# Angtian/VoGE

Measured on AMD Instinct MI355X. Metric: forward+backward frames/sec at 512^2, 50k Gaussians; ray-trace HBM GB/s vs peak, higher is better.
Workload: dtype f32; 1 GPU; cfg3_50k_512: 50000 random Gaussians (scalar sigmas), 512x512, K=40, max_point_per_bin=-1, fwd+bwd (grads to verts, sigmas, colors); launch=hip graph replay, 4 consecutive steps per graph launch, parallelism=1 gpu

## Files before the change

voge_amd/csrc/fragment_bwd.hip:

```cpp
#include "composite_core.h"

namespace voge {

#ifndef VOGE_FB_NE
#define VOGE_FB_NE 128
#endif
constexpr int kFbNE = VOGE_FB_NE;
#ifndef VOGE_FB_GW
#define VOGE_FB_GW 4
#endif
#ifndef VOGE_FB_GH
#define VOGE_FB_GH 3
#endif
constexpr int kFbGW = VOGE_FB_GW, kFbGH = VOGE_FB_GH, kFbG = kFbGW * kFbGH;
static_assert(kFbG <= 64 && (kFbGW & (kFbGW - 1)) == 0, "a group's pixels are the lanes of one wave; GW a power of two");
#ifdef VOGE_FB_TIMES
constexpr int kFbTimesWaves = 1 << 16;
__device__ unsigned long long g_fb_times[kFbTimesWaves][8];
__device__ unsigned long long g_fb_tab[kFbTimesWaves][4];
__device__ unsigned long long g_fb_wall[kFbTimesWaves][2];
#define FB_T0() const unsigned long long fb_w0_ = __builtin_amdgcn_s_memrealtime(); unsigned long long fb_t_ = __builtin_readcyclecounter(), fb_acc_[6] = {0, 0, 0, 0, 0, 0}
#define FB_TICK(i) do { const unsigned long long n_ = __builtin_readcyclecounter(); fb_acc_[i] += n_ - fb_t_; fb_t_ = n_; } while (0)
#define FB_TOUT() do { if (threadIdx.x == 0 && blockIdx.x < kFbTimesWaves) { for (int i_ = 0; i_ < 6; ++i_) g_fb_times[blockIdx.x][i_] = fb_acc_[i_]; g_fb_times[blockIdx.x][6] = 1ull; g_fb_wall[blockIdx.x][0] = fb_w0_; g_fb_wall[blockIdx.x][1] = __builtin_amdgcn_s_memrealtime(); } } while (0)
#else
#define FB_T0() do {} while (0)
#define FB_TICK(i) do {} while (0)
#define FB_TOUT() do {} while (0)
#endif

template <int NV4, int NS>
struct FragBwdLds {
  static constexpr int kRows = NS * 64 + 4 * kFbG;
  WaveTable<kFbNE, NV4> tab;
  float len[kRows], sp[kRows], E[kRows], u[kRows];
  float r[kRows];
  unsigned spare[kFbG];
};

#ifndef VOGE_FB_ABL
#define VOGE_FB_ABL 0
#endif
#ifndef VOGE_FB_WPE
#define VOGE_FB_WPE 4
#endif
template <int SRC, int C, int NS, typename OffT, bool ISO, bool NOAD, bool DIAG = false>
__global__ void __launch_bounds__(64) __attribute__((amdgpu_waves_per_eu(NS == 4 ? 2 : (ISO ? VOGE_FB_WPE : 3))))
fragment_bwd_kernel(const float4 *__restrict__ rec, const float *__restrict__ rays,
                        const float *__restrict__ colors, const int32_t *__restrict__ idx, const int32_t *__restrict__ cnt,
                        const float *__restrict__ weight, const float *__restrict__ act, const float *__restrict__ len,
                        const float *__restrict__ dsd, const float *__restrict__ rgb, const float *__restrict__ wsum,
                        const float *__restrict__ bg, const float thr, const float *__restrict__ g_img, const long gs_pix,
                        const long gs_c, const float *__restrict__ g_hitlen, const float occ,
                        const int P, const long nrows, const int W, const int K, const long Nattr,
                        float *__restrict__ acc ) {
  static_assert(NS == 2 || NS == 4, "a lane owns one or two aligned pairs of slots");
  static_assert(!DIAG || (!ISO && NOAD && C <= 4), "the per-axis form keeps no act / dsd");
  constexpr int NV4 = SRC == 0 ? (ISO ? 2 : (DIAG ? 3 : 4)) : (ISO ? 1 : (DIAG ? 2 : 3)), NACC = 4 * NV4;
  constexpr int NRC = ISO ? 1 : (DIAG ? 2 : 3);
  auto sum_add = [&](const int key, const int c, const float v) { unsafeAtomicAdd(acc + NACC * (size_t)key + c, v); };
  __shared__ __attribute__((aligned(16))) FragBwdLds<NV4, NS> L;
  float *const Llen = L.len, *const Lsp = L.sp, *const LE = L.E, *const Lu = L.u, *const LR = L.r;
  const int lane = threadIdx.x;
  FB_T0();
  const int blocks_x = (W + kFbGW - 1) / kFbGW;
  const long blk = blockIdx.x;
  const int x0 = (int)(blk % blocks_x) * kFbGW;
  const long y0 = (blk / blocks_x) * kFbGH;
  const bool vec = (K % NS) == 0;
  const int gx = x0 + (lane & (kFbGW - 1));
  const long gy = y0 + lane / kFbGW;
  const bool pv = lane < kFbG && gx < W && gy < nrows;
  const int lead_g = pv ? min(K, max(0, cnt[gy * W + gx])) : 0;
  const int need = (lead_g + NS - 1) / NS;
  const int incl = wave_incl_scan(need, lane);
  if (__builtin_amdgcn_readlane(incl, 63) == 0) return;
  wt_clear(L.tab, lane);
  int pc = 0, off = 0;
  while (pc < kFbG) {
    PackLane pk;
    int npm;
    const int pe = pack_round(need, incl, kFbG, lane, pc, off, pk, npm);
    off = __builtin_amdgcn_readlane(incl, pe - 1);
    pc = pe;
    if (npm == 0) continue;
    FB_TICK(0);
    const bool on = pk.p >= 0;
    const int q = on ? lane - pk.s0 : 0, LP = on ? pk.np : 1;
    const int lead = __shfl(lead_g, on ? pk.p : 0, 64);
    const int k0 = NS * q;
    const OffT pix = on ? (OffT)((y0 + pk.p / kFbGW) * W + x0 + (pk.p & (kFbGW - 1))) : (OffT)0;
    const OffT fb = (pix * (OffT)K + (OffT)k0) * (OffT)4;
    const int r0 = NS * pk.s0 + 4 * pk.ord, RS = NS * LP + 4;
    const int d0 = on ? r0 + 2 + k0 : 2;
    int id[NS];
    float wv[NS], lm[NS], sm[NS], em[NS], gwv[NS];
    bool live[NS];
#pragma unroll
    for (int a = 0; a < NS; ++a) {
      id[a] = -1; wv[a] = 0.f; lm[a] = VOGE_SENT_LEN; sm[a] = 1e-5f; em[a] = 0.f; gwv[a] = 0.f;
      live[a] = on && (k0 + a < lead);
    }
    const float3 dv = at_bytes<float3>(rays, pix * (OffT)12);
    const float dx = on ? dv.x : 0.f, dy = on ? dv.y : 0.f, dz = on ? dv.z : 0.f;
    float4 rc[NS][NRC];
    float av[NS], dv2[NS];
#pragma unroll
    for (int a = 0; a < NS; ++a) { av[a] = 0.f; dv2[a] = 0.f; }
    {
      int idr[NS];
      float wr[NS], lr[NS], ar[NS], dr[NS], gr_[NS];
#pragma unroll
      for (int a = 0; a < NS; ++a) { idr[a] = -1; wr[a] = 0.f; lr[a] = VOGE_SENT_LEN; ar[a] = 0.f; dr[a] = 0.f; gr_[a] = 0.f; }
      const bool gw_wide = SRC == 1 && g_img != nullptr && vec && gs_c == 1 && gs_pix == (long)K;
      if (vec) {
#pragma unroll
        for (int h2 = 0; h2 < NS / 2; ++h2) {
          const OffT fo = fb + (OffT)(8 * h2);
          const int2 i2 = at_bytes<int2>(idx, fo);
          const v2f w2 = at_bytes<v2f>(weight, fo), l2 = at_bytes<v2f>(len, fo);
          idr[2 * h2] = i2.x; idr[2 * h2 + 1] = i2.y; wr[2 * h2] = w2.x; wr[2 * h2 + 1] = w2.y; lr[2 * h2] = l2.x; lr[2 * h2 + 1] = l2.y;
          if (!NOAD) {
            const v2f a2 = at_bytes<v2f>(act, fo), d2 = at_bytes<v2f>(dsd, fo);
            ar[2 * h2] = a2.x; ar[2 * h2 + 1] = a2.y; dr[2 * h2] = d2.x; dr[2 * h2 + 1] = d2.y;
          }
          if (gw_wide) {
            const v2f g2 = at_bytes<v2f>(g_img, fo);
            gr_[2 * h2] = g2.x; gr_[2 * h2 + 1] = g2.y;
          }
        }
      } else {
#pragma unroll
        for (int a = 0; a < NS; ++a) {
          const OffT fo = (pix * (OffT)K + (OffT)min(k0 + a, K - 1)) * (OffT)4;
          idr[a] = at_bytes<int>(idx, fo); wr[a] = at_bytes<float>(weight, fo); lr[a] = at_bytes<float>(len, fo);
          if (!NOAD) { ar[a] = at_bytes<float>(act, fo); dr[a] = at_bytes<float>(dsd, fo); }
        }
      }
      if (SRC == 1 && g_img != nullptr && !gw_wide) {
#pragma unroll
        for (int a = 0; a < NS; ++a) gr_[a] = g_img[(long)pix * gs_pix + (long)min(k0 + a, K - 1) * gs_c];
      }
#pragma unroll
      for (int a = 0; a < NS; ++a) {
        if (live[a]) { id[a] = idr[a]; wv[a] = wr[a]; lm[a] = lr[a]; av[a] = ar[a]; dv2[a] = dr[a]; gwv[a] = gr_[a]; }
      }
    }
    float gr[4] = {0.f, 0.f, 0.f, 0.f}, g_sum_w = 0.0f;
    float px_ws = 0.f, px_rgb[4] = {0.f, 0.f, 0.f, 0.f}, px_g[4] = {0.f, 0.f, 0.f, 0.f};
    if (SRC == 2) {
      if (g_img != nullptr) px_g[0] = g_img[(long)pix * gs_pix];
      px_ws = at_bytes<float>(wsum, pix * (OffT)4);
      px_rgb[0] = at_bytes<float>(rgb, pix * (OffT)4);
      if (bg != nullptr) px_g[1] = at_bytes<float>(bg, pix * (OffT)4);
    }
    if (SRC == 0) {
#pragma unroll
      for (int c = 0; c < C; ++c) px_g[c] = g_img[(long)pix * gs_pix + c * gs_c];
      if (wsum != nullptr) px_ws = at_bytes<float>(wsum, pix * (OffT)4);
      if (bg != nullptr) {
// ... 162 lines not shown
      if (go) {
        if (ISO) {
          const float mx = rc[a][0].x, my = rc[a][0].y, mz = rc[a][0].z, aa = rc[a][0].w;
          const float t = fmaf(mz, dz, fmaf(my, dy, mx * dx)) * idn;
          float vx = fmaf(-t, dx, mx), vy = fmaf(-t, dy, my), vz = fmaf(-t, dz, mz);
          {
            const float rr = fmaf(vz, dz, fmaf(vy, dy, vx * dx)) * idn;
            vx = fmaf(-rr, dx, vx); vy = fmaf(-rr, dy, vy); vz = fmaf(-rr, dz, vz);
          }
          const float c1 = gl[a] * idn, c2 = 2.0f * aa * ga[a];
          val[0] = make_float4(fmaf(c1, dx, c2 * vx), fmaf(c1, dy, c2 * vy), fmaf(c1, dz, c2 * vz),
                               fmaf(ga[a], fmaf(vz, vz, fmaf(vy, vy, vx * vx)), gd[a] * dn2));
        } else if (DIAG) {
          const float4 r0 = rc[a][0], r1 = rc[a][NRC - 1];
          const float mx = r0.x, my = r0.y, mz = r0.z;
          const float adx = r0.w * dx, ady = r1.x * dy, adz = r1.y * dz;
          const float ksk = fmaf(dz, adz, fmaf(dy, ady, dx * adx)), msk = fmaf(mz, adz, fmaf(my, ady, mx * adx));
          const float ik = __builtin_amdgcn_rcpf(ksk);
          const float t = msk * ik;
          float vx = fmaf(-t, dx, mx), vy = fmaf(-t, dy, my), vz = fmaf(-t, dz, mz);
          {
            const float rr = fmaf(vz, adz, fmaf(vy, ady, vx * adx)) * ik;
            vx = fmaf(-rr, dx, vx); vy = fmaf(-rr, dy, vy); vz = fmaf(-rr, dz, vz);
          }
          const float avx = r0.w * vx, avy = r1.x * vy, avz = r1.y * vz;
          const float c1 = gl[a] * ik, g_a = ga[a], g_d = gd[a];
          const float o0 = fmaf(c1, adx, g_a * (avx + avx)), o1 = fmaf(c1, ady, g_a * (avy + avy)), o2 = fmaf(c1, adz, g_a * (avz + avz));
          const float o3 = fmaf(g_a, vx * vx, fmaf(g_d, dx * dx, c1 * (vx * dx)));
          const float o4 = fmaf(g_a, vy * vy, fmaf(g_d, dy * dy, c1 * (vy * dy)));
          const float o5 = fmaf(g_a, vz * vz, fmaf(g_d, dz * dz, c1 * (vz * dz)));
          val[0] = make_float4(o0, o1, o2, o3);
          if (SRC == 0) {
            val[NV4 >= 2 ? 1 : 0] = make_float4(o4, o5, wv[a] * gr[0], wv[a] * gr[1]);
            val[NV4 >= 3 ? 2 : 0] = make_float4(wv[a] * gr[2], wv[a] * gr[3], 0.f, 0.f);
          } else {
            val[NV4 >= 2 ? 1 : 0] = make_float4(o4, o5, 0.f, 0.f);
          }
        } else {
          const float4 r0 = rc[a][0], r1 = rc[a][NRC == 3 ? 1 : 0], r2 = rc[a][NRC == 3 ? 2 : 0];
          const float mx = r0.x, my = r0.y, mz = r0.z;
          const float A[9] = {r0.w, r1.x, r1.y, r1.z, r1.w, r2.x, r2.y, r2.z, r2.w};
          const float adx = fmaf(A[2], dz, fmaf(A[1], dy, A[0] * dx)), ady = fmaf(A[5], dz, fmaf(A[4], dy, A[3] * dx)),
                      adz = fmaf(A[8], dz, fmaf(A[7], dy, A[6] * dx));
          const float tdx = fmaf(A[6], dz, fmaf(A[3], dy, A[0] * dx)), tdy = fmaf(A[7], dz, fmaf(A[4], dy, A[1] * dx)),
                      tdz = fmaf(A[8], dz, fmaf(A[5], dy, A[2] * dx));
          const float ksk = fmaf(dz, adz, fmaf(dy, ady, dx * adx)), msk = fmaf(mz, adz, fmaf(my, ady, mx * adx));
          const float ik = __builtin_amdgcn_rcpf(ksk);
          const float t = msk * ik;
          float vx = fmaf(-t, dx, mx), vy = fmaf(-t, dy, my), vz = fmaf(-t, dz, mz);
          {
            const float rr = fmaf(vz, adz, fmaf(vy, ady, vx * adx)) * ik;
            vx = fmaf(-rr, dx, vx); vy = fmaf(-rr, dy, vy); vz = fmaf(-rr, dz, vz);
          }
          const float avx = fmaf(A[2], vz, fmaf(A[1], vy, A[0] * vx)), avy = fmaf(A[5], vz, fmaf(A[4], vy, A[3] * vx)),
                      avz = fmaf(A[8], vz, fmaf(A[7], vy, A[6] * vx));
          const float tvx = fmaf(A[6], vz, fmaf(A[3], vy, A[0] * vx)), tvy = fmaf(A[7], vz, fmaf(A[4], vy, A[1] * vx)),
                      tvz = fmaf(A[8], vz, fmaf(A[5], vy, A[2] * vx));
          const float c1 = gl[a] * ik, g_a = ga[a], g_d = gd[a];
          float o[12];
          o[0] = fmaf(c1, adx, g_a * (avx + tvx + t * (tdx - adx)));
          o[1] = fmaf(c1, ady, g_a * (avy + tvy + t * (tdy - ady)));
          o[2] = fmaf(c1, adz, g_a * (avz + tvz + t * (tdz - adz)));
          const float d[3] = {dx, dy, dz}, v[3] = {vx, vy, vz};
#pragma unroll
          for (int i = 0; i < 3; ++i)
#pragma unroll
            for (int c = 0; c < 3; ++c)
              o[3 + 3 * i + c] = fmaf(g_a, fmaf(v[i], v[c], t * (d[i] * v[c] - v[i] * d[c])), fmaf(g_d, d[i] * d[c], c1 * (v[i] * d[c])));
          val[0] = make_float4(o[0], o[1], o[2], o[3]);
          val[NV4 >= 3 ? 1 : 0] = make_float4(o[4], o[5], o[6], o[7]);
          val[NV4 >= 3 ? 2 : 0] = make_float4(o[8], o[9], o[10], o[11]);
        }
        if (SRC == 0 && !DIAG) val[NV4 - 1] = make_float4(wv[a] * gr[0], wv[a] * gr[1], wv[a] * gr[2], wv[a] * gr[3]);
        go = false;
#pragma unroll
        for (int r = 0; r < NV4; ++r) go = go || (val[r].x != 0.f || val[r].y != 0.f || val[r].z != 0.f || val[r].w != 0.f);
      }
      if (PAIR) {
#pragma unroll
        for (int r = 0; r < NV4; ++r) valp[PAIR ? a : 0][r] = val[r];
        gop[a] = go;
        continue;
      }
      if (!__any(go)) continue;
      FB_TICK(3);
#if VOGE_FB_ABL & 1
      if (go && val[0].x == 1.2345f && val[NV4 - 1].y == 3.21f) acc[id[a]] = val[0].w + val[NV4 - 1].x;
      continue;
#endif
      const int slot = wt_find(L.tab, id[a], go);
#ifdef VOGE_FB_TIMES
      {
        lds_vint *owner = lds_volatile(L.tab.owner);
        bool pending = go && slot >= 0;
        const unsigned long long m0 = __ballot(pending);
        unsigned rounds = 0;
        while (__any(pending)) {
          if (pending) owner[slot] = lane;
          if (pending && owner[slot] == lane) pending = false;
          ++rounds;
        }
        if (lane == 0 && blockIdx.x < kFbTimesWaves) {
          g_fb_tab[blockIdx.x][0] += 1; g_fb_tab[blockIdx.x][1] += rounds; g_fb_tab[blockIdx.x][2] += (unsigned)__popcll(m0);
        }
      }
#endif
      wt_add(L.tab, slot, val, go && slot >= 0, lane);
      if (go && slot < 0) {
#pragma unroll
        for (int r = 0; r < NV4; ++r) {
          const float o[4] = {val[r].x, val[r].y, val[r].z, val[r].w};
#pragma unroll
          for (int c = 0; c < 4; ++c) sum_add(id[a], 4 * r + c, o[c]);
        }
      }
      FB_TICK(4);
    }
    if (PAIR && __any(gop[0] | gop[1])) {
      FB_TICK(3);
      int slot0, slot1;
      wt_find2(L.tab, id[0], gop[0], id[NS - 1], gop[1], slot0, slot1);
      wt_add2_by_group(L.tab, slot0, valp[0], gop[0] && slot0 >= 0, slot1, valp[PAIR ? 1 : 0], gop[1] && slot1 >= 0, pk.ord);
#pragma unroll
      for (int a = 0; a < 2; ++a) {
        const int sl = a == 0 ? slot0 : slot1;
        if (gop[a] && sl < 0) {
#pragma unroll
          for (int r = 0; r < NV4; ++r) {
            const float o[4] = {valp[PAIR ? a : 0][r].x, valp[PAIR ? a : 0][r].y, valp[PAIR ? a : 0][r].z, valp[PAIR ? a : 0][r].w};
#pragma unroll
            for (int c = 0; c < 4; ++c) sum_add(id[a == 0 ? 0 : NS - 1], 4 * r + c, o[c]);
          }
        }
      }
      FB_TICK(4);
    }
  }
  FB_TICK(0);
  {
    constexpr int EPI = 64 / NACC;
    const int e = lane / NACC, c = lane - e * NACC;
    const float *vals = reinterpret_cast<const float *>(L.tab.vals);
    const int n = wt_compact(L.tab, lane);
    const lds_vint *list = lds_volatile(L.tab.owner);
    for (int i = e; i < n && e < EPI; i += EPI) {
      const int s = list[i];
      sum_add(L.tab.keys[s], c, vals[s * NACC + c]);
    }
  }
  FB_TICK(5);
  FB_TOUT();
}

__global__ void __launch_bounds__(256)
fragment_bwd_finish_kernel(const float *__restrict__ acc, const int S, const float *__restrict__ a_in, const int P, const int N,
                           const int B, const IsoView view, const int C, const long Nattr, float *__restrict__ g_mus,
                           float *__restrict__ g_a, float *__restrict__ g_colors) {
  const int g = blockIdx.x * blockDim.x + threadIdx.x;
  if (g_colors != nullptr && g < Nattr) {
    for (int c = 0; c < C; ++c) g_colors[(size_t)g * C + c] = (g < P) ? acc[S * (size_t)g + 4 + c] : 0.0f;
  }
  const int n_out = view.shared ? N : P;
  if (g >= n_out || g_mus == nullptr) return;
  float4 v = *reinterpret_cast<const float4 *>(acc + S * (size_t)g);
  if (view.shared)
    for (int b = 1; b < B; ++b) {
      const float4 w = *reinterpret_cast<const float4 *>(acc + S * ((size_t)b * N + g));
      v.x += w.x; v.y += w.y; v.z += w.z; v.w += w.w;
    }
  g_mus[3 * (size_t)g] = v.x; g_mus[3 * (size_t)g + 1] = v.y; g_mus[3 * (size_t)g + 2] = v.z;
  float ga = v.w;
  if (view.mode == 1) ga = 2.0f * ga;
  else if (view.mode == 2) { const float s = a_in[g]; ga = -2.0f * ga / (s * s); }
  g_a[g] = ga;
}

__global__ void __launch_bounds__(256)
fragment_bwd_pack_kernel(const float *__restrict__ mus, const float *__restrict__ isg, const int P, float4 *__restrict__ rec,
                         float4 *__restrict__ acc, const int S4 ) {
  const int g = blockIdx.x * blockDim.x + threadIdx.x;
  if (g >= P) return;
  for (int q = 0; q < S4; ++q) acc[S4 * (size_t)g + q] = make_float4(0.f, 0.f, 0.f, 0.f);
  const float *m = mus + 3 * (size_t)g, *A = isg + 9 * (size_t)g;
  rec[3 * (size_t)g + 0] = make_float4(m[0], m[1], m[2], A[0]);
  rec[3 * (size_t)g + 1] = make_float4(A[1], A[2], A[3], A[4]);
  rec[3 * (size_t)g + 2] = make_float4(A[5], A[6], A[7], A[8]);
}
__global__ void __launch_bounds__(256)
fragment_bwd_finish_general_kernel(const float *__restrict__ acc, const int S, const int P, const int C, const long Nattr,
                                   float *__restrict__ g_mus, float *__restrict__ g_isg, float *__restrict__ g_colors) {
  const long t = (long)blockIdx.x * blockDim.x + threadIdx.x;
  const long g = t >> 4;
  const int c = (int)(t & 15);
  if ((g >= P && g >= Nattr) || c >= S) return;
  const float v = (g < P) ? acc[g * S + c] : 0.0f;
  if (c < 3) { if (g < P && g_mus != nullptr) g_mus[3 * g + c] = v; }
  else if (c < 12) { if (g < P && g_isg != nullptr) g_isg[9 * g + (c - 3)] = v; }
  else if (c - 12 < C && g < Nattr && g_colors != nullptr) g_colors[g * C + (c - 12)] = v;
}

__global__ void __launch_bounds__(256)
fragment_act_dsd_iso_kernel(const float4 *__restrict__ rec, const float *__restrict__ rays, const int32_t *__restrict__ idx,
                            const float *__restrict__ len, const int32_t *__restrict__ cnt, const long npix, const int K,
                            const int P, float *__restrict__ act, float *__restrict__ dsd) {
  const long t = (long)blockIdx.x * blockDim.x + threadIdx.x;
  if (t >= npix * K) return;
  const long pix = t / K;
  const int k = (int)(t - pix * K);
  float a = VOGE_SENT_ACT, d = 0.0f;
  const int id = idx[t];
  if (k < cnt[pix] && id >= 0 && id < P) {
    const float4 r = rec[id];
    const float dx = rays[pix * 3], dy = rays[pix * 3 + 1], dz = rays[pix * 3 + 2];
    const PairOut o = pair_eval_iso_at(r.x, r.y, r.z, r.w, len[t], dx, dy, dz, (dx * dx + dy * dy) + dz * dz);
    a = o.act; d = o.dsd;
  }
  act[t] = a; dsd[t] = d;
}

}

using namespace voge;

#ifdef VOGE_FB_TIMES
extern "C" int voge_debug_fb_times(unsigned long long *out, int reset) {
  static unsigned long long host[voge::kFbTimesWaves][8];
  if (reset) {
    for (auto &row : host) for (auto &v : row) v = 0;
    return (int)hipMemcpyToSymbol(HIP_SYMBOL(voge::g_fb_times), host, sizeof(host));
  }
// ... 560 lines not shown
```

voge_amd/csrc/voge_common.h:

```cpp
#pragma once
#include <hip/hip_runtime.h>
#include <stdint.h>

#include <atomic>

#include "voge_hip.h"

#define VOGE_WAVE 64

#define VOGE_SENT_LEN 1e10f
#define VOGE_SENT_ACT 1e10f

namespace voge {

struct EvalRec {
  float s00, s11, s22, s01, s02, s12;
  float bx, by, bz;
  float kx, ky, kz;
};
static_assert(sizeof(EvalRec) == 48, "EvalRec must be 3 x float4");

__device__ __forceinline__ float fast_div(const float a, const float b) { return a * __builtin_amdgcn_rcpf(b); }

constexpr uint32_t kIsoFlag = 0x7fc0a150u;

struct IsoView {
  const float *origin;
  int shared, mode;
  int cam_origin = 0;
  int gen_kind = 0, sigma_shared = 0;
  const float *quats = nullptr;
  int ori_mode = 1;
};
__device__ __forceinline__ float iso_view_a(const float s, const int mode) {
  return mode == 1 ? 2.0f * s : (mode == 2 ? 2.0f / s : s);
}

__device__ __forceinline__ bool quat_usable(const float qw, const float qx, const float qy, const float qz) {
  const float n2 = qw * qw + qx * qx + qy * qy + qz * qz;
  return n2 > 0.0f && n2 < INFINITY;
}

template <typename T>
__device__ __forceinline__ void quat_rotation(const bool ok, const T qw, const T qx, const T qy, const T qz, T R[9], T qh[4], T &inv) {
  const T n2 = qw * qw + qx * qx + qy * qy + qz * qz;
  inv = ok ? (T)1 / sqrt(n2) : (T)0;
  const T w = ok ? qw * inv : (T)1, x = ok ? qx * inv : (T)0, y = ok ? qy * inv : (T)0, z = ok ? qz * inv : (T)0;
  qh[0] = w; qh[1] = x; qh[2] = y; qh[3] = z;
  R[0] = (T)1 - (T)2 * (y * y + z * z); R[1] = (T)2 * (x * y - w * z); R[2] = (T)2 * (x * z + w * y);
  R[3] = (T)2 * (x * y + w * z); R[4] = (T)1 - (T)2 * (x * x + z * z); R[5] = (T)2 * (y * z - w * x);
  R[6] = (T)2 * (x * z - w * y); R[7] = (T)2 * (y * z + w * x); R[8] = (T)1 - (T)2 * (x * x + y * y);
}

struct PairOut {
  float len, act, dsd;
};

__device__ __forceinline__ PairOut pair_eval_iso(const float mx, const float my, const float mz, const float a,
                                                 const float dx, const float dy, const float dz,
                                                 const float qxx, const float qyy, const float qzz) {
  PairOut o;
  const float dn2 = qxx + qyy + qzz;
  const float md = fmaf(mz, dz, fmaf(my, dy, mx * dx));
  const float t = fast_div(md, dn2) + 0.0f;
  const float vx = fmaf(-t, dx, mx);
  const float vy = fmaf(-t, dy, my);
  const float vz = fmaf(-t, dz, mz);
  o.len = t;
  o.act = a * fmaf(vz, vz, fmaf(vy, vy, vx * vx));
  o.dsd = a * dn2;
  return o;
}

__device__ __forceinline__ PairOut pair_eval_iso_at(const float mx, const float my, const float mz, const float a,
                                                    const float t, const float dx, const float dy, const float dz,
                                                    const float dn2) {
  PairOut o;
  const float vx = fmaf(-t, dx, mx);
  const float vy = fmaf(-t, dy, my);
  const float vz = fmaf(-t, dz, mz);
  o.len = t;
  o.act = a * fmaf(vz, vz, fmaf(vy, vy, vx * vx));
  o.dsd = a * dn2;
  return o;
}

__device__ __forceinline__ PairOut pair_eval_gen(const float mx, const float my, const float mz,
// ... 607 lines not shown
  quad = ConeRec{VOGE_LANE(cn.ax, 4), VOGE_LANE(cn.ay, 4), VOGE_LANE(cn.az, 4), VOGE_LANE(cn.cs, 4), VOGE_LANE(cn.sn, 4), VOGE_LANE(okf, 4), 0.f, 0.f};
}

__device__ __forceinline__ bool cull_has_ell(const float4 c) { return (__float_as_uint(c.w) & 1u) != 0u && c.w > 0.0f && c.w < 3e38f; }

__device__ __forceinline__ float ell_support(const float4 e0, const float4 e1, const float nx, const float ny, const float nz) {
  const float d = fmaf(e0.z * nz, nz, fmaf(e0.y * ny, ny, e0.x * nx * nx));
  const float o = fmaf(e1.y * ny, nz, fmaf(e1.x * nx, nz, e0.w * nx * ny));
  const float h2 = fmaxf(fmaf(2.0f, o, d), 0.0f) + e1.z;
  return fmaf(sqrtf(h2), 1.0f + 1e-5f, e1.w);
}

__device__ __forceinline__ bool cone_keep_ell(const float4 c, const float4 e0, const float4 e1, const Cone &k) {
  if (!k.ok) return true;
  const float p = fmaf(c.z, k.az, fmaf(c.y, k.ay, c.x * k.ax));
  const float rx = fmaf(-p, k.ax, c.x), ry = fmaf(-p, k.ay, c.y), rz = fmaf(-p, k.az, c.z);
  const float q2 = fmaf(rz, rz, fmaf(ry, ry, rx * rx));
  if (!(q2 > 1e-24f)) return true;
  const float iq = __builtin_amdgcn_rsqf(q2);
  const float q = q2 * iq;
  const float ux = rx * iq, uy = ry * iq, uz = rz * iq;
  const float qc = q * k.cs, ps = p * k.sn;
  const float err = 4e-6f * (q + fabsf(p));
  bool sep = true;
#pragma unroll
  for (int s = 0; s < 2; ++s) {
    const float sg = s ? -k.sn : k.sn;
    const float nx = fmaf(-sg, k.ax, k.cs * ux), ny = fmaf(-sg, k.ay, k.cs * uy), nz = fmaf(-sg, k.az, k.cs * uz);
    const float g = (s ? qc + ps : qc - ps) - err;
    sep = sep && (g > ell_support(e0, e1, nx, ny, nz));
  }
  return !sep;
}

typedef __attribute__((address_space(3))) volatile int lds_vint;
typedef __attribute__((address_space(3))) volatile unsigned lds_vuint;
__device__ __forceinline__ lds_vint *lds_volatile(int *p) { return (lds_vint *)p; }
__device__ __forceinline__ const lds_vint *lds_volatile(const int *p) { return (const lds_vint *)p; }
__device__ __forceinline__ lds_vuint *lds_volatile(unsigned *p) { return (lds_vuint *)p; }
typedef __attribute__((address_space(3))) volatile float lds_vfloat;
__device__ __forceinline__ const lds_vfloat *lds_volatile(const float *p) { return (const lds_vfloat *)p; }

__device__ __forceinline__ void wave_lds_sync() {
  __builtin_amdgcn_fence(__ATOMIC_RELEASE, "wavefront");
  __builtin_amdgcn_wave_barrier();
  __builtin_amdgcn_fence(__ATOMIC_ACQUIRE, "wavefront");
}

template <int NE, int NV4>
struct WaveTable {
  int keys[NE];
  int owner[NE];
  float4 vals[NE * NV4];
};

template <int NE, int NV4>
__device__ __forceinline__ void wt_clear(WaveTable<NE, NV4> &t, const int lane) {
  for (int i = lane; i < NE; i += VOGE_WAVE) t.keys[i] = -1;
  for (int i = lane; i < NE * NV4; i += VOGE_WAVE) t.vals[i] = make_float4(0.f, 0.f, 0.f, 0.f);
}

constexpr int kWtProbe = 16;
template <int NE, int NV4>
__device__ __forceinline__ int wt_find(WaveTable<NE, NV4> &t, const int key, const bool want) {
  unsigned h = ((unsigned)key * 2654435761u) >> (32 - __builtin_ctz(NE));
  int slot = -1;
  bool pending = want;
#pragma unroll 1
  for (int pr = 0; pr < kWtProbe && __any(pending); ++pr) {
    if (pending) {
      const int old = atomicCAS(&t.keys[h], -1, key);
      if (old == -1 || old == key) {
        slot = (int)h;
        pending = false;
      } else {
        h = (h + 1) & (NE - 1);
      }
    }
  }
  return slot;
}

template <int NE, int NV4>
__device__ __forceinline__ void wt_find2(WaveTable<NE, NV4> &t, const int key0, const bool want0, const int key1, const bool want1,
                                         int &slot0, int &slot1) {
  unsigned h0 = ((unsigned)key0 * 2654435761u) >> (32 - __builtin_ctz(NE));
  unsigned h1 = ((unsigned)key1 * 2654435761u) >> (32 - __builtin_ctz(NE));
  slot0 = slot1 = -1;
  bool p0 = want0, p1 = want1;
#pragma unroll 1
  for (int pr = 0; pr < kWtProbe && __any(p0 | p1); ++pr) {
    int old0 = -2, old1 = -2;
    if (p0) old0 = atomicCAS(&t.keys[h0], -1, key0);
    if (p1) old1 = atomicCAS(&t.keys[h1], -1, key1);
    if (p0) {
      if (old0 == -1 || old0 == key0) { slot0 = (int)h0; p0 = false; } else h0 = (h0 + 1) & (NE - 1);
    }
    if (p1) {
      if (old1 == -1 || old1 == key1) { slot1 = (int)h1; p1 = false; } else h1 = (h1 + 1) & (NE - 1);
    }
  }
}

template <int NE, int NV4>
__device__ __forceinline__ void wt_add(WaveTable<NE, NV4> &t, const int slot, const float4 (&v)[NV4],
                                       const bool on, const int lane) {
  lds_vint *owner = lds_volatile(t.owner);
  bool pending = on;
#pragma unroll 1
  while (__any(pending)) {
    if (pending) owner[slot] = lane;
    if (pending && owner[slot] == lane) {
      float4 *dst = t.vals + slot * NV4;
#pragma unroll
      for (int q = 0; q < NV4; ++q) {
        float4 x = dst[q];
        x.x += v[q].x; x.y += v[q].y; x.z += v[q].z; x.w += v[q].w;
        dst[q] = x;
      }
      pending = false;
    }
  }
}

template <int NE, int NV4>
__device__ __forceinline__ void wt_add2_by_group(WaveTable<NE, NV4> &t, const int slot0, const float4 (&v0)[NV4], const bool on0,
                                                 const int slot1, const float4 (&v1)[NV4], const bool on1, const int ord) {
  bool pend = on0 | on1;
#pragma unroll 1
  for (int g = 0; __any(pend); ++g) {
    if (pend && ord == g) {
      if (on0) {
        float4 *dst = t.vals + slot0 * NV4;
#pragma unroll
        for (int q = 0; q < NV4; ++q) {
          float4 x = dst[q];
          x.x += v0[q].x; x.y += v0[q].y; x.z += v0[q].z; x.w += v0[q].w;
          dst[q] = x;
        }
      }
      if (on1) {
        float4 *dst = t.vals + slot1 * NV4;
#pragma unroll
        for (int q = 0; q < NV4; ++q) {
          float4 x = dst[q];
          x.x += v1[q].x; x.y += v1[q].y; x.z += v1[q].z; x.w += v1[q].w;
          dst[q] = x;
        }
      }
      pend = false;
    }
    wave_lds_sync();
  }
}

template <int NE, int NV4>
__device__ __forceinline__ int wt_compact(WaveTable<NE, NV4> &t, const int lane) {
  lds_vint *list = lds_volatile(t.owner);
  int n = 0;
#pragma unroll
  for (int base = 0; base < NE; base += VOGE_WAVE) {
    const bool occ = (base + lane < NE) && (t.keys[base + lane] >= 0);
    const unsigned long long m = __ballot(occ);
    if (occ) list[n + __popcll(m & ((1ull << lane) - 1ull))] = base + lane;
    n += __popcll(m);
  }
  return n;
}

__device__ __forceinline__ float row16_sum(float v) {
  v += __int_as_float(__builtin_amdgcn_update_dpp(0, __float_as_int(v), 0xB1, 0xF, 0xF, true));
  v += __int_as_float(__builtin_amdgcn_update_dpp(0, __float_as_int(v), 0x4E, 0xF, 0xF, true));
  v += __int_as_float(__builtin_amdgcn_update_dpp(0, __float_as_int(v), 0x141, 0xF, 0xF, true));
  v += __int_as_float(__builtin_amdgcn_update_dpp(0, __float_as_int(v), 0x140, 0xF, 0xF, true));
  return v;
}

__device__ __forceinline__ float seg_sum(float x, const int lane, const int seg) {
  const int r = lane % seg;
  for (int o = 1; o < seg; o <<= 1) {
    const float y = __shfl_down(x, o, VOGE_WAVE);
    if (r + o < seg) x += y;
  }
  return x;
}

__device__ __forceinline__ float seg_sum_key(float x, const int key, const int lane) {
#pragma unroll
  for (int o = 1; o < VOGE_WAVE; o <<= 1) {
    const float y = __shfl_down(x, o, VOGE_WAVE);
    const int k2 = __shfl_down(key, o, VOGE_WAVE);
    if (lane + o < VOGE_WAVE && k2 == key) x += y;
  }
  return x;
}

inline int launch_status() { return (int)hipGetLastError(); }

static __global__ void __launch_bounds__(256) voge_fill32_kernel(uint32_t *__restrict__ p, const size_t n, const uint32_t value) {
  const size_t i = ((size_t)blockIdx.x * blockDim.x + threadIdx.x) * 4;
  if (i + 3 < n && (reinterpret_cast<uintptr_t>(p + i) & 15) == 0) {
    *reinterpret_cast<uint4 *>(p + i) = make_uint4(value, value, value, value);
  } else {
    for (size_t j = i; j < n && j < i + 4; ++j) p[j] = value;
  }
}
inline hipError_t voge_fill_async(void *p, const int byte_value, const size_t bytes, hipStream_t st) {
  if (bytes == 0 || p == nullptr) return hipSuccess;
  const uint32_t b = (uint32_t)(byte_value & 0xff), v = b | (b << 8) | (b << 16) | (b << 24);
  const size_t n = bytes / 4;
  hipLaunchKernelGGL(voge_fill32_kernel, dim3((unsigned)((n + 1023) / 1024)), dim3(256), 0, st, reinterpret_cast<uint32_t *>(p), n, v);
  return hipGetLastError();
}

struct DynLdsCache {
  std::atomic<size_t> set[16];
  DynLdsCache() { for (auto &v : set) v.store(0); }
};
inline int ensure_dynamic_lds(const void *func, const size_t lds, DynLdsCache &cache) {
  int dev = 0;
  if (hipGetDevice(&dev) != hipSuccess || dev < 0 || dev >= 16) dev = -1;
  if (dev >= 0 && lds <= cache.set[dev].load(std::memory_order_relaxed)) return 0;
  const hipError_t e = hipFuncSetAttribute(func, hipFuncAttributeMaxDynamicSharedMemorySize, (int)lds);
  if (e != hipSuccess) return (int)e;
  if (dev >= 0) cache.set[dev].store(lds, std::memory_order_relaxed);
  return 0;
}

}
```

Baseline: 4264 frames/s.

## Use a directory-indexed dense accumulator table for paired-slot backward accumulation

```diff
diff --git a/voge_amd/csrc/fragment_bwd.hip b/voge_amd/csrc/fragment_bwd.hip
--- a/voge_amd/csrc/fragment_bwd.hip
+++ b/voge_amd/csrc/fragment_bwd.hip
@@ -6,6 +6,16 @@
 #define VOGE_FB_NE 128
 #endif
 constexpr int kFbNE = VOGE_FB_NE;
+#ifndef VOGE_FB_ND
+#define VOGE_FB_ND 256
+#endif
+#ifndef VOGE_FB_ND_FRAME
+#define VOGE_FB_ND_FRAME 512
+#endif
+#ifndef VOGE_FB_NEV
+#define VOGE_FB_NEV 96
+#endif
+constexpr int kFbND = VOGE_FB_ND, kFbNDFrame = VOGE_FB_ND_FRAME, kFbNEV = VOGE_FB_NEV;
 #ifndef VOGE_FB_GW
 #define VOGE_FB_GW 4
 #endif
@@ -28,13 +38,12 @@
 #define FB_TOUT() do {} while (0)
 #endif
 
-template <int NV4, int NS>
+template <int NV4, int NS, int ND>
 struct FragBwdLds {
   static constexpr int kRows = NS * 64 + 4 * kFbG;
-  WaveTable<kFbNE, NV4> tab;
+  std::conditional_t<NS == 2, WaveDirTable<ND, kFbNEV, NV4>, WaveTable<kFbNE, NV4>> tab;
   float len[kRows], sp[kRows], E[kRows], u[kRows];
   float r[kRows];
-  unsigned spare[kFbG];
 };
 
 #ifndef VOGE_FB_ABL
@@ -58,7 +67,8 @@
   constexpr int NV4 = SRC == 0 ? (ISO ? 2 : (DIAG ? 3 : 4)) : (ISO ? 1 : (DIAG ? 2 : 3)), NACC = 4 * NV4;
   constexpr int NRC = ISO ? 1 : (DIAG ? 2 : 3);
   auto sum_add = [&](const int key, const int c, const float v) { unsafeAtomicAdd(acc + NACC * (size_t)key + c, v); };
-  __shared__ __attribute__((aligned(16))) FragBwdLds<NV4, NS> L;
+  constexpr int ND = (SRC == 0 && ISO && C == 3) ? kFbNDFrame : kFbND;
+  __shared__ __attribute__((aligned(16))) FragBwdLds<NV4, NS, ND> L;
   float *const Llen = L.len, *const Lsp = L.sp, *const LE = L.E, *const Lu = L.u, *const LR = L.r;
   const int lane = threadIdx.x;
   FB_T0();
@@ -74,7 +84,7 @@
   const int need = (lead_g + NS - 1) / NS;
   const int incl = wave_incl_scan(need, lane);
   if (__builtin_amdgcn_readlane(incl, 63) == 0) return;
-  wt_clear(L.tab, lane);
+  if constexpr (NS == 2) wd_clear(L.tab, lane); else wt_clear(L.tab, lane);
   int pc = 0, off = 0;
   while (pc < kFbG) {
     PackLane pk;
@@ -403,6 +413,7 @@
         gop[a] = go;
         continue;
       }
+      if constexpr (!PAIR) {
       if (!__any(go)) continue;
       FB_TICK(3);
 #if VOGE_FB_ABL & 1
@@ -436,11 +447,15 @@
         }
       }
       FB_TICK(4);
-    }
-    if (PAIR && __any(gop[0] | gop[1])) {
+      }
+    }
+    if constexpr (PAIR) if (__any(gop[0] | gop[1])) {
       FB_TICK(3);
+#if VOGE_FB_ABL & 1
+      if (gop[0] && gop[1] && valp[0][0].x == 1.2345f && valp[PAIR ? 1 : 0][NV4 - 1].y == 3.21f) acc[id[0]] = valp[0][NV4 - 1].w + valp[PAIR ? 1 : 0][0].x;
+#else
       int slot0, slot1;
-      wt_find2(L.tab, id[0], gop[0], id[NS - 1], gop[1], slot0, slot1);
+      wd_find2(L.tab, id[0], gop[0], id[NS - 1], gop[1], lane, slot0, slot1);
       wt_add2_by_group(L.tab, slot0, valp[0], gop[0] && slot0 >= 0, slot1, valp[PAIR ? 1 : 0], gop[1] && slot1 >= 0, pk.ord);
 #pragma unroll
       for (int a = 0; a < 2; ++a) {
@@ -454,6 +469,7 @@
           }
         }
       }
+#endif
       FB_TICK(4);
     }
   }
@@ -462,11 +478,16 @@
     constexpr int EPI = 64 / NACC;
     const int e = lane / NACC, c = lane - e * NACC;
     const float *vals = reinterpret_cast<const float *>(L.tab.vals);
-    const int n = wt_compact(L.tab, lane);
-    const lds_vint *list = lds_volatile(L.tab.owner);
-    for (int i = e; i < n && e < EPI; i += EPI) {
-      const int s = list[i];
-      sum_add(L.tab.keys[s], c, vals[s * NACC + c]);
+    if constexpr (NS == 2) {
+      const int n = wd_count(L.tab);
+      for (int i = e; i < n && e < EPI; i += EPI) sum_add(L.tab.ekey[i], c, vals[i * NACC + c]);
+    } else {
+      const int n = wt_compact(L.tab, lane);
+      const lds_vint *list = lds_volatile(L.tab.owner);
+      for (int i = e; i < n && e < EPI; i += EPI) {
+        const int s = list[i];
+        sum_add(L.tab.keys[s], c, vals[s * NACC + c]);
+      }
     }
   }
   FB_TICK(5);
diff --git a/voge_amd/csrc/voge_common.h b/voge_amd/csrc/voge_common.h
--- a/voge_amd/csrc/voge_common.h
+++ b/voge_amd/csrc/voge_common.h
@@ -3,6 +3,7 @@
 #include <stdint.h>
 
 #include <atomic>
+#include <type_traits>
 
 #include "voge_hip.h"
 
@@ -776,27 +777,6 @@
 }
 
 template <int NE, int NV4>
-__device__ __forceinline__ void wt_find2(WaveTable<NE, NV4> &t, const int key0, const bool want0, const int key1, const bool want1,
-                                         int &slot0, int &slot1) {
-  unsigned h0 = ((unsigned)key0 * 2654435761u) >> (32 - __builtin_ctz(NE));
-  unsigned h1 = ((unsigned)key1 * 2654435761u) >> (32 - __builtin_ctz(NE));
-  slot0 = slot1 = -1;
-  bool p0 = want0, p1 = want1;
-#pragma unroll 1
-  for (int pr = 0; pr < kWtProbe && __any(p0 | p1); ++pr) {
-    int old0 = -2, old1 = -2;
-    if (p0) old0 = atomicCAS(&t.keys[h0], -1, key0);
-    if (p1) old1 = atomicCAS(&t.keys[h1], -1, key1);
-    if (p0) {
-      if (old0 == -1 || old0 == key0) { slot0 = (int)h0; p0 = false; } else h0 = (h0 + 1) & (NE - 1);
-    }
-    if (p1) {
-      if (old1 == -1 || old1 == key1) { slot1 = (int)h1; p1 = false; } else h1 = (h1 + 1) & (NE - 1);
-    }
-  }
-}
-
-template <int NE, int NV4>
 __device__ __forceinline__ void wt_add(WaveTable<NE, NV4> &t, const int slot, const float4 (&v)[NV4],
                                        const bool on, const int lane) {
   lds_vint *owner = lds_volatile(t.owner);
@@ -817,35 +797,98 @@
   }
 }
 
-template <int NE, int NV4>
-__device__ __forceinline__ void wt_add2_by_group(WaveTable<NE, NV4> &t, const int slot0, const float4 (&v0)[NV4], const bool on0,
+template <class Tab, int NV4>
+__device__ __forceinline__ void wt_add2_by_group(Tab &t, const int slot0, const float4 (&v0)[NV4], const bool on0,
                                                  const int slot1, const float4 (&v1)[NV4], const bool on1, const int ord) {
   bool pend = on0 | on1;
+  float4 *const d0 = t.vals + (on0 ? slot0 : 0) * NV4, *const d1 = t.vals + (on1 ? slot1 : 0) * NV4;
 #pragma unroll 1
   for (int g = 0; __any(pend); ++g) {
     if (pend && ord == g) {
+      float4 x0[NV4], x1[NV4];
+#pragma unroll
+      for (int q = 0; q < NV4; ++q) { x0[q] = d0[q]; x1[q] = d1[q]; }
+#pragma unroll
+      for (int q = 0; q < NV4; ++q) {
+        x0[q].x += v0[q].x; x0[q].y += v0[q].y; x0[q].z += v0[q].z; x0[q].w += v0[q].w;
+        x1[q].x += v1[q].x; x1[q].y += v1[q].y; x1[q].z += v1[q].z; x1[q].w += v1[q].w;
+      }
       if (on0) {
-        float4 *dst = t.vals + slot0 * NV4;
-#pragma unroll
-        for (int q = 0; q < NV4; ++q) {
-          float4 x = dst[q];
-          x.x += v0[q].x; x.y += v0[q].y; x.z += v0[q].z; x.w += v0[q].w;
-          dst[q] = x;
-        }
+#pragma unroll
+        for (int q = 0; q < NV4; ++q) d0[q] = x0[q];
       }
       if (on1) {
-        float4 *dst = t.vals + slot1 * NV4;
-#pragma unroll
-        for (int q = 0; q < NV4; ++q) {
-          float4 x = dst[q];
-          x.x += v1[q].x; x.y += v1[q].y; x.z += v1[q].z; x.w += v1[q].w;
-          dst[q] = x;
-        }
+#pragma unroll
+        for (int q = 0; q < NV4; ++q) d1[q] = x1[q];
       }
       pend = false;
     }
     wave_lds_sync();
   }
+}
+
+constexpr unsigned kWdNone = 0xFFu;
+template <int ND, int NE, int NV4>
+struct WaveDirTable {
+  static_assert((ND & (ND - 1)) == 0 && ND >= 4 && ND <= 65536 && NE < (int)kWdNone, "directory: a power of two; entry indices are bytes");
+  float4 vals[NE * NV4];
+  int keys[ND];
+  int ekey[NE];
+  unsigned char eidx[ND];
+  int n;
+};
+
+template <int ND, int NE, int NV4>
+__device__ __forceinline__ void wd_clear(WaveDirTable<ND, NE, NV4> &t, const int lane) {
+  for (int i = lane; i < ND; i += VOGE_WAVE) t.keys[i] = -1;
+  for (int i = lane; i < NE * NV4; i += VOGE_WAVE) t.vals[i] = make_float4(0.f, 0.f, 0.f, 0.f);
+  if (lane == 0) t.n = 0;
+}
+template <int ND, int NE, int NV4>
+__device__ __forceinline__ int wd_count(const WaveDirTable<ND, NE, NV4> &t) { return min(t.n, NE); }
+
+template <int ND, int NE, int NV4>
+__device__ __forceinline__ void wd_find2(WaveDirTable<ND, NE, NV4> &t, const int key0, const bool want0, const int key1, const bool want1,
+                                         const int lane, int &e0, int &e1) {
+  constexpr int B = __builtin_ctz(ND);
+  constexpr unsigned kFound = 1u << 30, kClaimed = 1u << 31;
+  const unsigned m0 = (unsigned)key0 * 2654435761u, m1 = (unsigned)key1 * 2654435761u;
+  unsigned h0 = m0 >> (32 - B), h1 = m1 >> (32 - B);
+  const unsigned s0 = ((m0 >> (32 - 2 * B)) & (ND - 1)) | 1u, s1 = ((m1 >> (32 - 2 * B)) & (ND - 1)) | 1u;
+  bool p0 = want0, p1 = want1;
+  const int n = t.n;
+#pragma unroll 1
+  for (int pr = 0; pr < kWtProbe && __any(p0 | p1); ++pr) {
+    int old0 = -2, old1 = -2;
+    if (p0) old0 = atomicCAS(&t.keys[h0], -1, key0);
+    if (p1) old1 = atomicCAS(&t.keys[h1], -1, key1);
+    const bool hit0 = old0 == -1 || old0 == key0, hit1 = old1 == -1 || old1 == key1;
+    h0 = hit0 ? (h0 | (old0 == -1 ? (kFound | kClaimed) : kFound)) : (p0 ? ((h0 + s0) & (ND - 1)) : h0);
+    h1 = hit1 ? (h1 | (old1 == -1 ? (kFound | kClaimed) : kFound)) : (p1 ? ((h1 + s1) & (ND - 1)) : h1);
+    p0 = p0 && !hit0;
+    p1 = p1 && !hit1;
+  }
+  const bool c0 = (h0 & kClaimed) != 0, c1 = (h1 & kClaimed) != 0, f0 = (h0 & kFound) != 0, f1 = (h1 & kFound) != 0;
+  h0 &= ND - 1; h1 &= ND - 1;
+  const unsigned long long b0 = __ballot(c0), b1 = __ballot(c1);
+  if (b0 | b1) {
+    const unsigned long long below = (1ull << lane) - 1ull;
+    const int n0 = __popcll(b0);
+    const int i0 = n + __popcll(b0 & below), i1 = n + n0 + __popcll(b1 & below);
+    if (c0) {
+      t.eidx[h0] = (unsigned char)(i0 < NE ? (unsigned)i0 : kWdNone);
+      if (i0 < NE) t.ekey[i0] = key0;
+    }
+    if (c1) {
+      t.eidx[h1] = (unsigned char)(i1 < NE ? (unsigned)i1 : kWdNone);
+      if (i1 < NE) t.ekey[i1] = key1;
+    }
+    if (lane == 0) t.n = n + n0 + __popcll(b1);
+    wave_lds_sync();
+  }
+  const unsigned x0 = f0 ? (unsigned)t.eidx[h0] : kWdNone, x1 = f1 ? (unsigned)t.eidx[h1] : kWdNone;
+  e0 = x0 == kWdNone ? -1 : (int)x0;
+  e1 = x1 == kWdNone ? -1 : (int)x1;
 }
 
 template <int NE, int NV4>
```

After: 4354 frames/s (median of 6 runs). 1.02x the previous value.
